# tsunrise/r1cs-spartan

Measured on AMD Instinct MI355X. Metric: R1CS constraints proved/sec at 2^20, higher is better.
Workload: dtype bls12-381 Fr/Fq Montgomery (u32 limbs)

## Files before the change

### r1cs-spartan_amd/csrc/curve29.hpp

```cpp
#pragma once
#include "curve_dev.hpp"
#include "ff29.hpp"

namespace spx {

template <class S>
struct R29;
template <>
struct R29<Fq> {
    using T = F29;
    static DEV void unpack(F29& r, const Fq& s) { f29_unpack(r, s.v); }
    static DEV void pack(Fq& s, const F29& r) { f29_pack(s.v, r); }
};
template <>
struct R29<Fq2> {
    using T = F2_29;
    static DEV void unpack(F2_29& r, const Fq2& s) {
        f29_unpack(r.c0, s.c0.v);
        f29_unpack(r.c1, s.c1.v);
    }
    static DEV void pack(Fq2& s, const F2_29& r) {
        f29_pack(s.c0.v, r.c0);
        f29_pack(s.c1.v, r.c1);
    }
};

template <class F>
struct A29 {
    F x, y;
};
template <class F>
struct X29 {
    F x, y, zz, zzz;
};

template <class S>
DEV void ld29(A29<typename R29<S>::T>& r, const Aff<S>* p) {
    Aff<S> a;
    load_vec(a, p);
    R29<S>::unpack(r.x, a.x);
    R29<S>::unpack(r.y, a.y);
}
template <class S>
DEV void ld29(X29<typename R29<S>::T>& r, const Xyzz<S>* p) {
    Xyzz<S> a;
    load_vec(a, p);
    R29<S>::unpack(r.x, a.x);
    R29<S>::unpack(r.y, a.y);
    R29<S>::unpack(r.zz, a.zz);
    R29<S>::unpack(r.zzz, a.zzz);
}
template <class S>
DEV void st29(Xyzz<S>* p, const X29<typename R29<S>::T>& r) {
    Xyzz<S> a;
    R29<S>::pack(a.x, r.x);
    R29<S>::pack(a.y, r.y);
    R29<S>::pack(a.zz, r.zz);
    R29<S>::pack(a.zzz, r.zzz);
    store_vec(p, a);
}

template <class F>
DEV void x29_set_inf(X29<F>& p) {
    using O = Ops29<F>;
    O::one(p.x);
    O::one(p.y);
    O::zero(p.zz);
    O::zero(p.zzz);
}
template <class F>
DEV bool x29_is_inf(const X29<F>& p) {
    return Ops29<F>::is_zero_raw(p.zz);
}

template <class F>
DEV void x29_from_aff_dbl(X29<F>& r, const F& ax, const F& ay) {
    using O = Ops29<F>;
    F U, V, W, S, X2, M, t, s2;
    O::add(U, ay, ay);
    O::sqr(V, U);
    O::mul(W, U, V);
    O::mul(S, ax, V);
    O::sqr(X2, ax);
    O::add(M, X2, X2);
    O::add(M, M, X2);
    O::sqr(t, M);
    O::add(s2, S, S);
    O::template sub<4>(r.x, t, s2);
    O::template reduce<8>(r.x);
    O::template sub<2>(t, S, r.x);
    if constexpr (O::kFusedSum) {
        O::zero(s2);
        O::template sub<2>(s2, s2, W);
        O::mul_sum(r.y, M, t, s2, ay);
    } else {
        O::mul(t, M, t);
        O::mul(s2, W, ay);
        O::template sub<2>(r.y, t, s2);
        O::template reduce<4>(r.y);
    }
    r.zz = V;
    r.zzz = W;
}

template <class F>
DEV void x29_dbl(X29<F>& p) {
    using O = Ops29<F>;
    if (x29_is_inf(p)) return;
    F U, V, W, S, X2, M, t, s2;
    O::add(U, p.y, p.y);
    O::sqr(V, U);
    O::mul(W, U, V);
    O::mul(S, p.x, V);
    O::sqr(X2, p.x);
    O::add(M, X2, X2);
    O::add(M, M, X2);
    O::sqr(t, M);
    O::add(s2, S, S);
    F x3;
    O::template sub<4>(x3, t, s2);
    O::template reduce<8>(x3);
    O::template sub<2>(t, S, x3);
    if constexpr (O::kFusedSum) {
        O::zero(s2);
        O::template sub<2>(s2, s2, W);
        O::mul_sum(p.y, M, t, s2, p.y);
    } else {
        O::mul(t, M, t);
        O::mul(s2, W, p.y);
        O::template sub<2>(p.y, t, s2);
        O::template reduce<4>(p.y);
    }
    p.x = x3;
    O::mul(p.zz, V, p.zz);
    O::mul(p.zzz, W, p.zzz);
}

template <class F>
DEV void x29_madd(X29<F>& p, const F& ax, const F& ay_in, bool neg) {
    using O = Ops29<F>;
    F ay = ay_in;
    if (neg) {
        F z;
        O::zero(z);
        O::template sub<2>(ay, z, ay_in);
    }
    if (x29_is_inf(p)) {
        p.x = ax;
        p.y = ay;
        O::one(p.zz);
        O::one(p.zzz);
        return;
    }
    F U2, S2, P, R;
    O::mul(U2, ax, p.zz);
    O::mul(S2, ay, p.zzz);
    O::template sub<8>(P, U2, p.x);
    O::template sub<4>(R, S2, p.y);
    if (O::template zero_lt<16>(P)) {
        if (O::template zero_lt<8>(R))
            x29_from_aff_dbl(p, ax, ay);
        else
            x29_set_inf(p);
        return;
    }
    F PP, PPP, Q, t, w;
    O::template sqr_b<16>(PP, P);
    O::mul(PPP, P, PP);
    O::mul(Q, p.x, PP);
    O::sqr(t, R);
    O::template sub<2>(w, t, PPP);
    O::add(t, Q, Q);
    O::template sub<4>(w, w, t);
    O::template sub<8>(t, Q, w);
    O::zero(S2);
    O::template sub<4>(S2, S2, p.y);
    O::mul_sum(p.y, t, R, S2, PPP);
    p.x = w;
    O::mul(p.zz, p.zz, PP);
    O::mul(p.zzz, p.zzz, PPP);
}

template <class F>
DEV void x29_add(X29<F>& p, const X29<F>& q) {
    using O = Ops29<F>;
    if (x29_is_inf(q)) return;
    if (x29_is_inf(p)) {
        p = q;
        return;
    }
    F U1, U2, S1, S2, P, R;
    O::mul(U1, p.x, q.zz);
    O::mul(U2, q.x, p.zz);
    O::mul(S1, p.y, q.zzz);
    O::mul(S2, q.y, p.zzz);
    O::template sub<2>(P, U2, U1);
    O::template sub<2>(R, S2, S1);
    if (O::template zero_lt<4>(P)) {
        if (O::template zero_lt<4>(R))
            x29_dbl(p);
        else
            x29_set_inf(p);
        return;
    }
    F PP, PPP, Q, t, w;
    O::sqr(PP, P);
    O::mul(PPP, P, PP);
    O::mul(Q, U1, PP);
    O::sqr(t, R);
    O::template sub<2>(w, t, PPP);
    O::add(t, Q, Q);
    O::template sub<4>(w, w, t);
    O::template reduce<8>(w);
    O::template sub<2>(t, Q, w);
    if constexpr (O::kFusedSum) {
        F n;
        O::zero(n);
        O::template sub<2>(n, n, S1);
        O::mul_sum(p.y, R, t, n, PPP);
    } else {
        O::mul(t, R, t);
        O::mul(S1, S1, PPP);
        O::template sub<2>(p.y, t, S1);
        O::template reduce<4>(p.y);
    }
    p.x = w;
    O::mul(t, p.zz, q.zz);
    O::mul(p.zz, t, PP);
    O::mul(t, p.zzz, q.zzz);
    O::mul(p.zzz, t, PPP);
}

template <class F>
DEV void f29_map(F& r, const F& x, const uint32_t (&c)[14]);
template <>
DEV void f29_map<F29>(F29& r, const F29& x, const uint32_t (&c)[14]) {
    F29 k;
    f29_set(k, c);
    f29_mul(r, x, k);
    f29_canon(r);
}
template <>
DEV void f29_map<F2_29>(F2_29& r, const F2_29& x, const uint32_t (&c)[14]) {
    f29_map<F29>(r.c0, x.c0, c);
    f29_map<F29>(r.c1, x.c1, c);
}

}
```

### r1cs-spartan_amd/csrc/ff29.hpp

```cpp
#pragma once
#include <stdint.h>

#include <hip/hip_runtime.h>

#ifndef DEV
#define DEV __device__ __forceinline__
#endif

namespace spx {

struct F29 {
    uint32_t v[14];
};

struct Q29 {
    static constexpr int N = 14;
    static constexpr uint32_t M = (1u << 29) - 1;
    static constexpr uint32_t PINV = 0x1ffcfffdu;
    static constexpr uint32_t P[14] = {0x1fffaaab, 0x0ff7ffff, 0x14ffffee, 0x17fffd62, 0x0f6241ea, 0x09507b58, 0x0afd9cc3,
                                       0x109e70a2, 0x1764774b, 0x121a5d66, 0x12c6e9ed, 0x12ffcd34, 0x00111ea3, 0x0000000d};
    static constexpr uint32_t P2[14] = {0x1fff5556, 0x1fefffff, 0x09ffffdc, 0x0ffffac5, 0x1ec483d5, 0x12a0f6b0, 0x15fb3986,
                                        0x013ce144, 0x0ec8ee97, 0x0434bacd, 0x058dd3db, 0x05ff9a69, 0x00223d47, 0x0000001a};
    static constexpr uint32_t P4[14] = {0x1ffeaaac, 0x1fdfffff, 0x13ffffb9, 0x1ffff58a, 0x1d8907aa, 0x0541ed61, 0x0bf6730d,
                                        0x0279c289, 0x1d91dd2e, 0x0869759a, 0x0b1ba7b6, 0x0bff34d2, 0x00447a8e, 0x00000034};
    static constexpr uint32_t P8[14] = {0x1ffd5558, 0x1fbfffff, 0x07ffff73, 0x1fffeb15, 0x1b120f55, 0x0a83dac3, 0x17ece61a,
                                        0x04f38512, 0x1b23ba5c, 0x10d2eb35, 0x16374f6c, 0x17fe69a4, 0x0088f51c, 0x00000068};
    static constexpr uint32_t P16[14] = {0x1ffaaab0, 0x1f7fffff, 0x0ffffee7, 0x1fffd62a, 0x16241eab, 0x1507b587,
                                         0x0fd9cc34, 0x09e70a25, 0x164774b8, 0x01a5d66b, 0x0c6e9ed9, 0x0ffcd349,
                                         0x0111ea39, 0x000000d0};
    static constexpr uint32_t INV5555 = 0xfffcfffdu;
    static constexpr uint32_t ONE[14] = {0x03a9fb84, 0x0ba00690, 0x071288f1, 0x0f59bcc5, 0x126cb614, 0x0585bf36, 0x1b85ac3d,
                                         0x1cf856fa, 0x1891ecbd, 0x1a7eec05, 0x155a88f0, 0x0741ac6d, 0x1317c30f, 0x00000009};
    static constexpr uint32_t TO_R1[14] = {0x0002fffd, 0x10480000, 0x0300009d, 0x08001788, 0x158baebf, 0x0c2ba9e3, 0x1d157d22,
                                           0x0a6e0a4a, 0x0d77ce58, 0x1d12b763, 0x1701c6a5, 0x1501c926, 0x1f65ec3f, 0x0000000a};
    static constexpr uint32_t FROM_R1[14] = {0x1fddebbd, 0x1a4f5474, 0x0291f399, 0x14d03b3c, 0x0f6cad2c, 0x1b4cabca,
                                             0x1592827c, 0x021c6ac7, 0x1ec52a84, 0x16fd5ec4, 0x0c960da6, 0x0fd2af6b,
                                             0x13263591, 0x0000000b};
};

template <int K>
DEV constexpr uint32_t kp29(int i) {
    static_assert(K == 1 || K == 2 || K == 4 || K == 8 || K == 16, "multiple of p");
    return K == 1 ? Q29::P[i] : K == 2 ? Q29::P2[i] : K == 4 ? Q29::P4[i] : K == 8 ? Q29::P8[i] : Q29::P16[i];
}

DEV void f29_set(F29& r, const uint32_t (&c)[14]) {
#pragma unroll
    for (int i = 0; i < 14; ++i) r.v[i] = c[i];
}
DEV void f29_zero(F29& r) {
#pragma unroll
    for (int i = 0; i < 14; ++i) r.v[i] = 0;
}
DEV void f29_one(F29& r) { f29_set(r, Q29::ONE); }

DEV uint64_t f29_opaque(uint64_t x) {
    asm("" : "+v"(x));
    return x;
}

template <int NP>
DEV void f29_redc_sum(F29& r, const F29* const (&a)[NP], const F29* const (&b)[NP]) {
    uint32_t m[14], t[14];
    uint64_t carry = 0;
#pragma unroll
    for (int k = 0; k < 27; ++k) {
        const int lo = k < 14 ? 0 : k - 13, hi = k < 14 ? k : 13;
        uint64_t ch = 0;
#pragma unroll
        for (int i = lo; i <= hi; ++i) {
#pragma unroll
            for (int q = 0; q < NP; ++q) ch += (uint64_t)a[q]->v[i] * b[q]->v[k - i];
        }
#pragma unroll
        for (int i = lo; i <= (k < 14 ? k - 1 : 13); ++i) ch += (uint64_t)m[i] * Q29::P[k - i];
        uint64_t acc = ch + carry;
        if (k < 14) {
            m[k] = ((uint32_t)acc * Q29::PINV) & Q29::M;
            acc += (uint64_t)m[k] * Q29::P[0];
        } else {
            t[k - 14] = (uint32_t)acc & Q29::M;
        }
        carry = acc >> 29;
    }
    t[13] = (uint32_t)carry;
#pragma unroll
    for (int i = 0; i < 14; ++i) r.v[i] = t[i];
}

DEV void f29_redc_sum4(F29& r, const F29& a0, const F29& b0, const F29& a1, const F29& b1, const F29& a2,
                       const F29& b2, const F29& a3, const F29& b3) {
    uint32_t m[14], t[14];
    uint64_t carry = 0;
#pragma unroll
    for (int k = 0; k < 27; ++k) {
        const int lo = k < 14 ? 0 : k - 13, hi = k < 14 ? k : 13;
        uint64_t ca = 0, cb = 0;
#pragma unroll
        for (int i = lo; i <= hi; ++i) {
            ca += (uint64_t)a0.v[i] * b0.v[k - i];
            ca += (uint64_t)a1.v[i] * b1.v[k - i];
            cb += (uint64_t)a2.v[i] * b2.v[k - i];
            cb += (uint64_t)a3.v[i] * b3.v[k - i];
        }
#pragma unroll
        for (int i = lo; i <= (k < 14 ? k - 1 : 13); ++i) cb += (uint64_t)m[i] * Q29::P[k - i];
        ca = f29_opaque(ca);
        cb = f29_opaque(cb);
        uint64_t low = (ca & Q29::M) + (cb & Q29::M) + (carry & Q29::M);
        const uint64_t high = (ca >> 29) + (cb >> 29) + (carry >> 29);
        if (k < 14) {
            m[k] = ((uint32_t)low * Q29::PINV) & Q29::M;
            low += (uint64_t)m[k] * Q29::P[0];
        } else {
            t[k - 14] = (uint32_t)low & Q29::M;
        }
        carry = high + (low >> 29);
    }
    t[13] = (uint32_t)carry;
#pragma unroll
    for (int i = 0; i < 14; ++i) r.v[i] = t[i];
}

DEV void f29_mul(F29& r, const F29& a, const F29& b) {
    const F29* const pa[1] = {&a};
    const F29* const pb[1] = {&b};
    f29_redc_sum<1>(r, pa, pb);
}

DEV void f29_mul2(F29& r, const F29& a, const F29& b, const F29& c, const F29& d) {
    const F29* const pa[2] = {&a, &c};
    const F29* const pb[2] = {&b, &d};
    f29_redc_sum<2>(r, pa, pb);
}

DEV void f29_add(F29& r, const F29& a, const F29& b) {
    uint32_t c = 0;
#pragma unroll
    for (int i = 0; i < 13; ++i) {
        const uint32_t t = a.v[i] + b.v[i] + c;
        r.v[i] = t & Q29::M;
        c = t >> 29;
    }
    r.v[13] = a.v[13] + b.v[13] + c;
}

template <int K>
DEV void f29_sub(F29& r, const F29& a, const F29& b) {
    int32_t c = 0;
#pragma unroll
    for (int i = 0; i < 13; ++i) {
        const int32_t t = (int32_t)a.v[i] - (int32_t)b.v[i] + (int32_t)kp29<K>(i) + c;
        r.v[i] = (uint32_t)t & Q29::M;
        c = t >> 29;
    }
    r.v[13] = (uint32_t)((int32_t)a.v[13] - (int32_t)b.v[13] + (int32_t)kp29<K>(13) + c);
}

template <int K>
DEV void f29_csub(F29& x) {
    uint32_t d[14];
    int32_t c = 0;
#pragma unroll
    for (int i = 0; i < 13; ++i) {
        const int32_t t = (int32_t)x.v[i] - (int32_t)kp29<K>(i) + c;
        d[i] = (uint32_t)t & Q29::M;
        c = t >> 29;
    }
    const int32_t top = (int32_t)x.v[13] - (int32_t)kp29<K>(13) + c;
    d[13] = (uint32_t)top;
    const bool keep = top < 0;
#pragma unroll
    for (int i = 0; i < 14; ++i) x.v[i] = keep ? x.v[i] : d[i];
}

template <int K>
DEV void f29_reduce(F29& x) {
    if constexpr (K >= 16) f29_csub<8>(x);
    if constexpr (K >= 8) f29_csub<4>(x);
    if constexpr (K >= 4) f29_csub<2>(x);
}

template <int K>
DEV bool f29_eq_kp(const F29& x) {
    uint32_t acc = 0;
#pragma unroll
    for (int i = 0; i < 14; ++i) acc |= x.v[i] ^ kp29<K>(i);
    return acc == 0;
}
DEV bool f29_is_zero_raw(const F29& x) {
    uint32_t acc = 0;
#pragma unroll
    for (int i = 0; i < 14; ++i) acc |= x.v[i];
    return acc == 0;
}
DEV bool f29_zero2(const F29& x) { return f29_is_zero_raw(x) || f29_eq_kp<1>(x); }
DEV bool f29_zero4(const F29& x) {
    F29 y = x;
    f29_csub<2>(y);
    return f29_zero2(y);
}
template <int K>
DEV bool f29_zero_lt(const F29& x) {
    const uint32_t v0 = x.v[0];
    const bool cand = v0 == 0 || ((1u << 29) - v0) * Q29::INV5555 < (uint32_t)K;
    if (!cand) return false;
    F29 y = x;
    f29_reduce<K>(y);
    return f29_zero2(y);
}
DEV void f29_canon(F29& x) { f29_csub<1>(x); }

DEV void f29_unpack(F29& r, const uint32_t* w) {
#pragma unroll
    for (int i = 0; i < 14; ++i) {
        const int o = 29 * i, k = o >> 5, s = o & 31;
        uint32_t v = w[k] >> s;
        if (s + 29 > 32 && k + 1 < 12) v |= w[k + 1] << (32 - s);
        r.v[i] = v & Q29::M;
    }
}
DEV void f29_pack(uint32_t* w, const F29& x) {
#pragma unroll
    for (int k = 0; k < 12; ++k) w[k] = 0;
#pragma unroll
    for (int i = 0; i < 14; ++i) {
        const int o = 29 * i, k = o >> 5, s = o & 31;
        w[k] |= x.v[i] << s;
        if (s + 29 > 32 && k + 1 < 12) w[k + 1] |= x.v[i] >> (32 - s);
    }
}

struct F2_29 {
    F29 c0, c1;
};
DEV void f2_29_mul(F2_29& r, const F2_29& a, const F2_29& b) {
    F29 nb1, c0, c1;
    F29 z;
    f29_zero(z);
    f29_sub<8>(nb1, z, b.c1);
    f29_mul2(c0, a.c0, b.c0, a.c1, nb1);
    f29_mul2(c1, a.c0, b.c1, a.c1, b.c0);
    r.c0 = c0;
    r.c1 = c1;
}
template <int KB = 8>
DEV void f2_29_sqr(F2_29& r, const F2_29& a) {
    F29 s, d, t, c0, c1;
    f29_add(s, a.c0, a.c1);
    f29_sub<KB>(d, a.c0, a.c1);
    f29_add(t, a.c0, a.c0);
    f29_mul(c0, s, d);
    f29_mul(c1, t, a.c1);
    r.c0 = c0;
    r.c1 = c1;
}

template <class F>
struct Ops29;
template <>
struct Ops29<F29> {
    static constexpr bool kFusedSum = true;
    static DEV void mul(F29& r, const F29& a, const F29& b) { f29_mul(r, a, b); }
    static DEV void mul_sum(F29& r, const F29& a, const F29& b, const F29& c, const F29& d) { f29_mul2(r, a, b, c, d); }
    static DEV void sqr(F29& r, const F29& a) { f29_mul(r, a, a); }
    static DEV void add(F29& r, const F29& a, const F29& b) { f29_add(r, a, b); }
    template <int K>
    static DEV void sub(F29& r, const F29& a, const F29& b) {
        f29_sub<K>(r, a, b);
    }
    template <int K>
    static DEV void reduce(F29& x) {
        f29_reduce<K>(x);
    }
    static DEV bool zero2(const F29& x) { return f29_zero2(x); }
    static DEV bool zero4(const F29& x) { return f29_zero4(x); }
    template <int K>
    static DEV bool zero_lt(const F29& x) {
        return f29_zero_lt<K>(x);
    }
    template <int KB>
    static DEV void sqr_b(F29& r, const F29& a) {
        f29_mul(r, a, a);
    }
    static DEV bool is_zero_raw(const F29& x) { return f29_is_zero_raw(x); }
    static DEV void zero(F29& r) { f29_zero(r); }
    static DEV void one(F29& r) { f29_one(r); }
};
template <>
struct Ops29<F2_29> {
    static constexpr bool kFusedSum = false;
    static DEV void mul(F2_29& r, const F2_29& a, const F2_29& b) { f2_29_mul(r, a, b); }
    static DEV void mul_sum(F2_29& r, const F2_29& a, const F2_29& b, const F2_29& c, const F2_29& d) {
        F2_29 x, y;
        f2_29_mul(x, a, b);
        f2_29_mul(y, c, d);
        f29_add(r.c0, x.c0, y.c0);
        f29_add(r.c1, x.c1, y.c1);
    }
    static DEV void sqr(F2_29& r, const F2_29& a) { f2_29_sqr(r, a); }
    static DEV void add(F2_29& r, const F2_29& a, const F2_29& b) {
        f29_add(r.c0, a.c0, b.c0);
        f29_add(r.c1, a.c1, b.c1);
    }
    template <int K>
    static DEV void sub(F2_29& r, const F2_29& a, const F2_29& b) {
        f29_sub<K>(r.c0, a.c0, b.c0);
        f29_sub<K>(r.c1, a.c1, b.c1);
    }
    template <int K>
    static DEV void reduce(F2_29& x) {
        f29_reduce<K>(x.c0);
        f29_reduce<K>(x.c1);
    }
    static DEV bool zero2(const F2_29& x) { return f29_zero2(x.c0) && f29_zero2(x.c1); }
    static DEV bool zero4(const F2_29& x) { return f29_zero4(x.c0) && f29_zero4(x.c1); }
    template <int K>
    static DEV bool zero_lt(const F2_29& x) {
        return f29_zero_lt<K>(x.c0) && f29_zero_lt<K>(x.c1);
    }
    template <int KB>
    static DEV void sqr_b(F2_29& r, const F2_29& a) {
        f2_29_sqr<KB>(r, a);
    }
    static DEV bool is_zero_raw(const F2_29& x) { return f29_is_zero_raw(x.c0) && f29_is_zero_raw(x.c1); }
    static DEV void zero(F2_29& r) {
        f29_zero(r.c0);
        f29_zero(r.c1);
    }
    static DEV void one(F2_29& r) {
        f29_one(r.c0);
        f29_zero(r.c1);
    }
};

}
```

### r1cs-spartan_amd/csrc/fq2pair.hpp

```cpp
#pragma once
#include "ff29.hpp"

namespace spx {

struct FP29 {
    F29 v;
};

DEV bool pair_odd() { return (__lane_id() & 1) != 0; }
DEV uint32_t pair_swap(uint32_t x) {
    return (uint32_t)__builtin_amdgcn_update_dpp(0, (int)x, 0xB1, 0xF, 0xF, false);
}
DEV F29 pair_swap(const F29& a) {
    F29 r;
#pragma unroll
    for (int i = 0; i < 14; ++i) r.v[i] = pair_swap(a.v[i]);
    return r;
}
DEV bool pair_all(bool b) {
    const uint32_t x = b ? 1u : 0u;
    return (x & pair_swap(x)) != 0;
}
DEV F29 f29_select(bool c, const F29& a, const F29& b) {
    F29 r;
#pragma unroll
    for (int i = 0; i < 14; ++i) r.v[i] = c ? a.v[i] : b.v[i];
    return r;
}

DEV uint32_t pair_even(uint32_t x) { return (uint32_t)__builtin_amdgcn_update_dpp(0, (int)x, 0xA0, 0xF, 0xF, false); }
DEV uint32_t pair_odd_val(uint32_t x) { return (uint32_t)__builtin_amdgcn_update_dpp(0, (int)x, 0xF5, 0xF, 0xF, false); }

DEV constexpr uint32_t k16(int i) {
    return i == 0 ? Q29::P16[0] + (1u << 29) : i < 13 ? Q29::P16[i] + (1u << 29) - 1u : Q29::P16[13] - 1u;
}

struct FP29A {
    F29 v;
};

template <class P, bool kBorrowFree>
struct PairOps {
    static constexpr bool kFusedSum = kBorrowFree;
    static DEV void mul(P& r, const P& a, const P& b) {
        const bool odd = pair_odd();
        if constexpr (kBorrowFree) {
            const uint32_t msk = odd ? 0u : 0xffffffffu;
            F29 ap, y1, y2;
#pragma unroll
            for (int i = 0; i < 14; ++i) {
                ap.v[i] = pair_swap(a.v.v[i]);
                y1.v[i] = pair_even(b.v.v[i]);
                const uint32_t z = pair_odd_val(b.v.v[i]);
                y2.v[i] = (z ^ msk) + (msk & (k16(i) + 1u));
            }
            f29_mul2(r.v, a.v, y1, ap, y2);
        } else {
            const F29 ap = pair_swap(a.v), bp = pair_swap(b.v);
            F29 z, nbp;
            f29_zero(z);
            f29_sub<8>(nbp, z, bp);
            const F29 y1 = f29_select(odd, bp, b.v);
            const F29 y2 = f29_select(odd, b.v, nbp);
            f29_mul2(r.v, a.v, y1, ap, y2);
        }
    }
    static DEV void mul_sum(P& r, const P& a, const P& b, const P& c, const P& d) {
        if constexpr (kBorrowFree) {
            const bool odd = pair_odd();
            const uint32_t msk = odd ? 0u : 0xffffffffu;
            F29 ap, y1, y2, cp, z1, z2;
#pragma unroll
            for (int i = 0; i < 14; ++i) {
                ap.v[i] = pair_swap(a.v.v[i]);
                y1.v[i] = pair_even(b.v.v[i]);
                const uint32_t yb = pair_odd_val(b.v.v[i]);
                y2.v[i] = (yb ^ msk) + (msk & (k16(i) + 1u));
                cp.v[i] = pair_swap(c.v.v[i]);
                z1.v[i] = pair_even(d.v.v[i]);
                const uint32_t zd = pair_odd_val(d.v.v[i]);
                z2.v[i] = (zd ^ msk) + (msk & (k16(i) + 1u));
            }
            f29_redc_sum4(r.v, a.v, y1, ap, y2, c.v, z1, cp, z2);
        } else {
            P x, y;
            mul(x, a, b);
            mul(y, c, d);
            f29_add(r.v, x.v, y.v);
        }
    }
    template <int KB>
    static DEV void sqr_b(P& r, const P& a) {
        const bool odd = pair_odd();
        const F29 ap = pair_swap(a.v);
        if constexpr (kBorrowFree) {
            F29 d, x, y;
            f29_sub<KB>(d, a.v, ap);
#pragma unroll
            for (int i = 0; i < 14; ++i) {
                x.v[i] = odd ? ap.v[i] : a.v.v[i] + ap.v[i];
                y.v[i] = odd ? a.v.v[i] + a.v.v[i] : d.v[i];
            }
            f29_mul(r.v, x, y);
            return;
        }
        F29 s, d, x, y;
        f29_add(s, a.v, ap);
        f29_sub<KB>(d, a.v, ap);
        f29_add(x, ap, ap);
        y = f29_select(odd, a.v, d);
        x = f29_select(odd, x, s);
        f29_mul(r.v, x, y);
    }
    static DEV void sqr(P& r, const P& a) { sqr_b<8>(r, a); }
    static DEV void add(P& r, const P& a, const P& b) { f29_add(r.v, a.v, b.v); }
    template <int K>
    static DEV void sub(P& r, const P& a, const P& b) {
        f29_sub<K>(r.v, a.v, b.v);
    }
    template <int K>
    static DEV void reduce(P& x) {
        f29_reduce<K>(x.v);
    }
    static DEV bool zero2(const P& x) { return pair_all(f29_zero2(x.v)); }
    static DEV bool zero4(const P& x) { return pair_all(f29_zero4(x.v)); }
    template <int K>
    static DEV bool zero_lt(const P& x) {
        return pair_all(f29_zero_lt<K>(x.v));
    }
    static DEV bool is_zero_raw(const P& x) { return pair_all(f29_is_zero_raw(x.v)); }
    static DEV void zero(P& r) { f29_zero(r.v); }
    static DEV void one(P& r) {
        if (pair_odd())
            f29_zero(r.v);
        else
            f29_one(r.v);
    }
};
template <>
struct Ops29<FP29> : PairOps<FP29, false> {};
template <>
struct Ops29<FP29A> : PairOps<FP29A, true> {};

template <class P>
DEV void fp29_unpack(P& r, const Fq2& s) {
    f29_unpack(r.v, pair_odd() ? s.c1.v : s.c0.v);
}
template <class P>
DEV void fp29_ld(P& r, const Fq2* coord) {
    Fq w;
    load_vec(w, pair_odd() ? &coord->c1 : &coord->c0);
    f29_unpack(r.v, w.v);
}
template <class P>
DEV void fp29_st(Fq2* coord, const P& r) {
    Fq w;
    f29_pack(w.v, r.v);
    store_vec(pair_odd() ? &coord->c1 : &coord->c0, w);
}

}
```

Baseline: 64.73 million.

## Interleave paired Montgomery multiplications in XYZZ mixed addition for ILP

Adds dual-stream Montgomery reduction routines (mul_x2, sqr_x2, mul2_x2) that run two independent 29-bit-limb products through one interleaved CIOS scan. The mixed-add formula is regrouped so independent multiplications and squarings are issued pairwise. The paired-lane operand prep is simplified to one DPP swap plus selects instead of separate even/odd DPP broadcasts, and pair_swap now uses mov_dpp. The aim is more instruction-level parallelism and fewer DPP ops, at the cost of higher register pressure that could lower occupancy or cause spills.

```diff
diff --git a/r1cs-spartan_amd/csrc/curve29.hpp b/r1cs-spartan_amd/csrc/curve29.hpp
--- a/r1cs-spartan_amd/csrc/curve29.hpp
+++ b/r1cs-spartan_amd/csrc/curve29.hpp
@@ -153,8 +153,7 @@
         return;
     }
     F U2, S2, P, R;
-    O::mul(U2, ax, p.zz);
-    O::mul(S2, ay, p.zzz);
+    O::mul_x2(U2, ax, p.zz, S2, ay, p.zzz);
     O::template sub<8>(P, U2, p.x);
     O::template sub<4>(R, S2, p.y);
     if (O::template zero_lt<16>(P)) {
@@ -165,10 +164,8 @@
         return;
     }
     F PP, PPP, Q, t, w;
-    O::template sqr_b<16>(PP, P);
-    O::mul(PPP, P, PP);
-    O::mul(Q, p.x, PP);
-    O::sqr(t, R);
+    O::template sqr_x2<16, 8>(PP, P, t, R);
+    O::mul_x2(PPP, P, PP, Q, p.x, PP);
     O::template sub<2>(w, t, PPP);
     O::add(t, Q, Q);
     O::template sub<4>(w, w, t);
@@ -177,8 +174,7 @@
     O::template sub<4>(S2, S2, p.y);
     O::mul_sum(p.y, t, R, S2, PPP);
     p.x = w;
-    O::mul(p.zz, p.zz, PP);
-    O::mul(p.zzz, p.zzz, PPP);
+    O::mul_x2(p.zz, p.zz, PP, p.zzz, p.zzz, PPP);
 }
 
 template <class F>
diff --git a/r1cs-spartan_amd/csrc/ff29.hpp b/r1cs-spartan_amd/csrc/ff29.hpp
--- a/r1cs-spartan_amd/csrc/ff29.hpp
+++ b/r1cs-spartan_amd/csrc/ff29.hpp
@@ -134,6 +134,100 @@
     f29_redc_sum<2>(r, pa, pb);
 }
 
+template <class Prod2>
+DEV void f29_redc_scan_x2(F29& r0, F29& r1, const Prod2& prod2) {
+    uint32_t m0[14], t0[14], m1[14], t1[14];
+    uint64_t c0 = 0, c1 = 0;
+#pragma unroll
+    for (int k = 0; k < 27; ++k) {
+        const int lo = k < 14 ? 0 : k - 13;
+        uint64_t x0 = c0, x1 = c1;
+        prod2(k, x0, x1);
+#pragma unroll
+        for (int i = lo; i <= (k < 14 ? k - 1 : 13); ++i) {
+            x0 = f29_opaque(x0 + (uint64_t)m0[i] * Q29::P[k - i]);
+            x1 = f29_opaque(x1 + (uint64_t)m1[i] * Q29::P[k - i]);
+        }
+        if (k < 14) {
+            m0[k] = ((uint32_t)x0 * Q29::PINV) & Q29::M;
+            m1[k] = ((uint32_t)x1 * Q29::PINV) & Q29::M;
+            x0 += (uint64_t)m0[k] * Q29::P[0];
+            x1 += (uint64_t)m1[k] * Q29::P[0];
+        } else {
+            t0[k - 14] = (uint32_t)x0 & Q29::M;
+            t1[k - 14] = (uint32_t)x1 & Q29::M;
+        }
+        c0 = x0 >> 29;
+        c1 = x1 >> 29;
+    }
+    t0[13] = (uint32_t)c0;
+    t1[13] = (uint32_t)c1;
+#pragma unroll
+    for (int i = 0; i < 14; ++i) {
+        r0.v[i] = t0[i];
+        r1.v[i] = t1[i];
+    }
+}
+template <int NP>
+DEV void f29_redc_sum_x2(F29& r0, F29& r1, const F29* const (&a0)[NP], const F29* const (&b0)[NP],
+                         const F29* const (&a1)[NP], const F29* const (&b1)[NP]) {
+    f29_redc_scan_x2(r0, r1, [&](int k, uint64_t& x0, uint64_t& x1) {
+        const int lo = k < 14 ? 0 : k - 13, hi = k < 14 ? k : 13;
+#pragma unroll
+        for (int i = lo; i <= hi; ++i) {
+#pragma unroll
+            for (int q = 0; q < NP; ++q) {
+                x0 = f29_opaque(x0 + (uint64_t)a0[q]->v[i] * b0[q]->v[k - i]);
+                x1 = f29_opaque(x1 + (uint64_t)a1[q]->v[i] * b1[q]->v[k - i]);
+            }
+        }
+    });
+}
+DEV void f29_sqr_x2(F29& r0, const F29& a0, F29& r1, const F29& a1) {
+    uint32_t d0[14], d1[14];
+#pragma unroll
+    for (int i = 0; i < 14; ++i) {
+        d0[i] = a0.v[i] << 1;
+        d1[i] = a1.v[i] << 1;
+    }
+    F29 x, y;
+    f29_redc_scan_x2(x, y, [&](int k, uint64_t& x0, uint64_t& x1) {
+        const int lo = k < 14 ? 0 : k - 13;
+        if (k % 2 == 0) {
+            x0 = f29_opaque(x0 + (uint64_t)a0.v[k / 2] * a0.v[k / 2]);
+            x1 = f29_opaque(x1 + (uint64_t)a1.v[k / 2] * a1.v[k / 2]);
+        }
+#pragma unroll
+        for (int i = lo; 2 * i < k; ++i) {
+            x0 = f29_opaque(x0 + (uint64_t)a0.v[i] * d0[k - i]);
+            x1 = f29_opaque(x1 + (uint64_t)a1.v[i] * d1[k - i]);
+        }
+    });
+    r0 = x;
+    r1 = y;
+}
+DEV void f29_mul_x2(F29& r0, const F29& a0, const F29& b0, F29& r1, const F29& a1, const F29& b1) {
+    const F29* const pa0[1] = {&a0};
+    const F29* const pb0[1] = {&b0};
+    const F29* const pa1[1] = {&a1};
+    const F29* const pb1[1] = {&b1};
+    F29 x, y;
+    f29_redc_sum_x2<1>(x, y, pa0, pb0, pa1, pb1);
+    r0 = x;
+    r1 = y;
+}
+DEV void f29_mul2_x2(F29& r0, const F29& a0, const F29& b0, const F29& c0, const F29& d0, F29& r1, const F29& a1,
+                     const F29& b1, const F29& c1, const F29& d1) {
+    const F29* const pa0[2] = {&a0, &c0};
+    const F29* const pb0[2] = {&b0, &d0};
+    const F29* const pa1[2] = {&a1, &c1};
+    const F29* const pb1[2] = {&b1, &d1};
+    F29 x, y;
+    f29_redc_sum_x2<2>(x, y, pa0, pb0, pa1, pb1);
+    r0 = x;
+    r1 = y;
+}
+
 DEV void f29_add(F29& r, const F29& a, const F29& b) {
     uint32_t c = 0;
 #pragma unroll
@@ -264,6 +358,13 @@
     static DEV void mul(F29& r, const F29& a, const F29& b) { f29_mul(r, a, b); }
     static DEV void mul_sum(F29& r, const F29& a, const F29& b, const F29& c, const F29& d) { f29_mul2(r, a, b, c, d); }
     static DEV void sqr(F29& r, const F29& a) { f29_mul(r, a, a); }
+    static DEV void mul_x2(F29& r0, const F29& a0, const F29& b0, F29& r1, const F29& a1, const F29& b1) {
+        f29_mul_x2(r0, a0, b0, r1, a1, b1);
+    }
+    template <int K0, int K1>
+    static DEV void sqr_x2(F29& r0, const F29& a0, F29& r1, const F29& a1) {
+        f29_sqr_x2(r0, a0, r1, a1);
+    }
     static DEV void add(F29& r, const F29& a, const F29& b) { f29_add(r, a, b); }
     template <int K>
     static DEV void sub(F29& r, const F29& a, const F29& b) {
@@ -299,6 +400,15 @@
         f29_add(r.c1, x.c1, y.c1);
     }
     static DEV void sqr(F2_29& r, const F2_29& a) { f2_29_sqr(r, a); }
+    static DEV void mul_x2(F2_29& r0, const F2_29& a0, const F2_29& b0, F2_29& r1, const F2_29& a1, const F2_29& b1) {
+        f2_29_mul(r0, a0, b0);
+        f2_29_mul(r1, a1, b1);
+    }
+    template <int K0, int K1>
+    static DEV void sqr_x2(F2_29& r0, const F2_29& a0, F2_29& r1, const F2_29& a1) {
+        f2_29_sqr<K0>(r0, a0);
+        f2_29_sqr<K1>(r1, a1);
+    }
     static DEV void add(F2_29& r, const F2_29& a, const F2_29& b) {
         f29_add(r.c0, a.c0, b.c0);
         f29_add(r.c1, a.c1, b.c1);
diff --git a/r1cs-spartan_amd/csrc/fq2pair.hpp b/r1cs-spartan_amd/csrc/fq2pair.hpp
--- a/r1cs-spartan_amd/csrc/fq2pair.hpp
+++ b/r1cs-spartan_amd/csrc/fq2pair.hpp
@@ -8,9 +8,7 @@
 };
 
 DEV bool pair_odd() { return (__lane_id() & 1) != 0; }
-DEV uint32_t pair_swap(uint32_t x) {
-    return (uint32_t)__builtin_amdgcn_update_dpp(0, (int)x, 0xB1, 0xF, 0xF, false);
-}
+DEV uint32_t pair_swap(uint32_t x) { return (uint32_t)__builtin_amdgcn_mov_dpp((int)x, 0xB1, 0xF, 0xF, true); }
 DEV F29 pair_swap(const F29& a) {
     F29 r;
 #pragma unroll
@@ -28,9 +26,6 @@
     return r;
 }
 
-DEV uint32_t pair_even(uint32_t x) { return (uint32_t)__builtin_amdgcn_update_dpp(0, (int)x, 0xA0, 0xF, 0xF, false); }
-DEV uint32_t pair_odd_val(uint32_t x) { return (uint32_t)__builtin_amdgcn_update_dpp(0, (int)x, 0xF5, 0xF, 0xF, false); }
-
 DEV constexpr uint32_t k16(int i) {
     return i == 0 ? Q29::P16[0] + (1u << 29) : i < 13 ? Q29::P16[i] + (1u << 29) - 1u : Q29::P16[13] - 1u;
 }
@@ -42,18 +37,20 @@
 template <class P, bool kBorrowFree>
 struct PairOps {
     static constexpr bool kFusedSum = kBorrowFree;
+    static DEV void prep(F29& y1, F29& y2, const F29& b, bool odd) {
+        const F29 bp = pair_swap(b);
+#pragma unroll
+        for (int i = 0; i < 14; ++i) {
+            y1.v[i] = odd ? bp.v[i] : b.v[i];
+            y2.v[i] = odd ? b.v[i] : k16(i) - bp.v[i];
+        }
+    }
     static DEV void mul(P& r, const P& a, const P& b) {
         const bool odd = pair_odd();
         if constexpr (kBorrowFree) {
-            const uint32_t msk = odd ? 0u : 0xffffffffu;
-            F29 ap, y1, y2;
-#pragma unroll
-            for (int i = 0; i < 14; ++i) {
-                ap.v[i] = pair_swap(a.v.v[i]);
-                y1.v[i] = pair_even(b.v.v[i]);
-                const uint32_t z = pair_odd_val(b.v.v[i]);
-                y2.v[i] = (z ^ msk) + (msk & (k16(i) + 1u));
-            }
+            const F29 ap = pair_swap(a.v);
+            F29 y1, y2;
+            prep(y1, y2, b.v, odd);
             f29_mul2(r.v, a.v, y1, ap, y2);
         } else {
             const F29 ap = pair_swap(a.v), bp = pair_swap(b.v);
@@ -65,22 +62,47 @@
             f29_mul2(r.v, a.v, y1, ap, y2);
         }
     }
+    static DEV void mul_x2(P& r0, const P& a0, const P& b0, P& r1, const P& a1, const P& b1) {
+        if constexpr (kBorrowFree) {
+            const bool odd = pair_odd();
+            const F29 ap0 = pair_swap(a0.v), ap1 = pair_swap(a1.v);
+            F29 y1, y2, z1, z2;
+            prep(y1, y2, b0.v, odd);
+            prep(z1, z2, b1.v, odd);
+            f29_mul2_x2(r0.v, a0.v, y1, ap0, y2, r1.v, a1.v, z1, ap1, z2);
+        } else {
+            mul(r0, a0, b0);
+            mul(r1, a1, b1);
+        }
+    }
+    template <int K0, int K1>
+    static DEV void sqr_x2(P& r0, const P& a0, P& r1, const P& a1) {
+        if constexpr (kBorrowFree) {
+            const bool odd = pair_odd();
+            const F29 ap0 = pair_swap(a0.v), ap1 = pair_swap(a1.v);
+            F29 d0, d1, x0, y0, x1, y1;
+            f29_sub<K0>(d0, a0.v, ap0);
+            f29_sub<K1>(d1, a1.v, ap1);
+#pragma unroll
+            for (int i = 0; i < 14; ++i) {
+                x0.v[i] = odd ? ap0.v[i] : a0.v.v[i] + ap0.v[i];
+                y0.v[i] = odd ? a0.v.v[i] + a0.v.v[i] : d0.v[i];
+                x1.v[i] = odd ? ap1.v[i] : a1.v.v[i] + ap1.v[i];
+                y1.v[i] = odd ? a1.v.v[i] + a1.v.v[i] : d1.v[i];
+            }
+            f29_mul_x2(r0.v, x0, y0, r1.v, x1, y1);
+        } else {
+            sqr_b<K0>(r0, a0);
+            sqr_b<K1>(r1, a1);
+        }
+    }
     static DEV void mul_sum(P& r, const P& a, const P& b, const P& c, const P& d) {
         if constexpr (kBorrowFree) {
             const bool odd = pair_odd();
-            const uint32_t msk = odd ? 0u : 0xffffffffu;
-            F29 ap, y1, y2, cp, z1, z2;
-#pragma unroll
-            for (int i = 0; i < 14; ++i) {
-                ap.v[i] = pair_swap(a.v.v[i]);
-                y1.v[i] = pair_even(b.v.v[i]);
-                const uint32_t yb = pair_odd_val(b.v.v[i]);
-                y2.v[i] = (yb ^ msk) + (msk & (k16(i) + 1u));
-                cp.v[i] = pair_swap(c.v.v[i]);
-                z1.v[i] = pair_even(d.v.v[i]);
-                const uint32_t zd = pair_odd_val(d.v.v[i]);
-                z2.v[i] = (zd ^ msk) + (msk & (k16(i) + 1u));
-            }
+            const F29 ap = pair_swap(a.v), cp = pair_swap(c.v);
+            F29 y1, y2, z1, z2;
+            prep(y1, y2, b.v, odd);
+            prep(z1, z2, d.v, odd);
             f29_redc_sum4(r.v, a.v, y1, ap, y2, c.v, z1, cp, z2);
         } else {
             P x, y;
```

After: 66.00 million, median of 6. 1.02x the previous value.
